# jianwang-mpi/GlobalEgoMocap

Hardware: AMD Instinct MI355X
Metric: optimised windows/sec (10-frame, 15-joint) (higher is better)
Workload: dtype f32

## Files before the change

### globalegomocap_amd/csrc/gem_internal.h

```cpp
#pragma once
#if defined(__HIP_DEVICE_COMPILE__) && !defined(GEM_NO_PACKED_FP32)
#error "compile with: -Xclang -target-feature -Xclang -packed-fp32-ops -DGEM_NO_PACKED_FP32 (__graft_entry__.NO_PACKED_FP32)"
#endif

#include <hip/hip_runtime.h>
#include <stdint.h>
#include <atomic>
#include <set>
#include <string>
#include <vector>

#include "../../include/gem_hip.h"

namespace gem {

constexpr int PAD = 64;
constexpr float LEAKY_SLOPE = 0.01f;
constexpr double BN_EPS = 1e-5;
constexpr int MAX_HIST = 128;
constexpr int MAXJ_ERR = GEM_MAX_JOINTS;
constexpr int N_LOG = 1 << 16;
constexpr int TRACE_ROUNDS = 64;

inline int pad64(int x) { return (x + PAD - 1) / PAD * PAD; }
// ... 88 lines not shown
    int *perm2 = nullptr, *slot_of2 = nullptr;
    int* n_log = nullptr;
    long log_pos = 0;
    int done_phase = 3;
    int dbg_slots = -1, dbg_B = 0, dbg_round = 0;
    long dbg_log0 = 0;
    std::vector<void*> allocs;
};

enum Repack {
    REPACK_NONE = 0,
    REPACK_KERNEL = 1,
    REPACK_FUSED = 2,
    REPACK_ATOMIC = 3
};

struct RoundSet {
    int* n_active = nullptr;
    int* perm = nullptr;
    int* slot_of = nullptr;
    int *next_perm = nullptr, *next_slot_of = nullptr, *next_count = nullptr;
    long log_idx = -1;
    double* trace = nullptr;
};

struct GemmOpts {
    const RoundSet* rs = nullptr;
    const int* row_map = nullptr;
    SlabSrc* defer = nullptr;
    int* repack_log = nullptr;
    GemmOpts() {}
    GemmOpts(std::nullptr_t) {}
    GemmOpts(const RoundSet* rs_, const int* row_map_, SlabSrc* defer_ = nullptr, int* repack_log_ = nullptr)
        : rs(rs_), row_map(row_map_), defer(defer_), repack_log(repack_log_) {}
};

template <typename T>
inline int dev_alloc(std::vector<void*>& owner, T** p, size_t n) {
    void* q = nullptr;
    if (!hip_ok(hipMalloc(&q, (n ? n : 1) * sizeof(T)), "hipMalloc")) return 1;
    owner.push_back(q);
    *p = static_cast<T*>(q);
    return hip_ok(hipMemset(q, 0, (n ? n : 1) * sizeof(T)), "hipMemset") ? 0 : 1;
}
template <typename T>
inline int upload(std::vector<void*>& owner, T** p, const std::vector<T>& v) {
// ... 122 lines not shown
        const DynSplit d = dyn_split(*s.m_dev, 64, s.CT, s.dyn_W, s.n_tiles, s.ldc);
        nslab = d.SK;
        stride = d.slab;
    }
}
bool rows_can_fuse_compaction(const gem_handle* h, const Layer& L, int lda, int ldc, int B, bool slabs);
int launch_splitk_reduce(gem_handle* h, int epi, int nslab, size_t slab, const float* bias, const float* aux, float* C, int M, int N,
                         int ldc, const int* m_dev, hipStream_t s, int dyn_W = 0, int n_tiles = 0);
int launch_gemm_bf16(gem_handle* h, const Layer& L, int epi, int nprod, const float* A, int lda, const float* aux, float* Cout,
                     int ldc, int M, int T, hipStream_t s, const GemmOpts& o);

enum Narrow {
    NARROW_BATCHED = 0,
    NARROW_TAIL_F32 = 1,
    NARROW_TAIL_BF16 = 2
};
struct Route {
    int precision = 0;
    Narrow narrow = NARROW_BATCHED;
    bool front = false;
    int tail_wgs = 0;
    int tail_cap = 0;
    Repack repack = REPACK_KERNEL;
};
enum Call { CALL_DECODE = 0, CALL_EVALUATE = 1, CALL_ROUNDS = 2 };
Route plan_route(const gem_handle* h, int stage, int B, Call call);

struct EnergyArgs;
int evaluate_bf16(gem_handle* h, const Route& rt, int stage, int B, const EnergyArgs& ea, hipStream_t s, bool forward_only, const RoundSet* rs,
                  SlabSrc* grad);
int launch_f32_to_bf16(const float* src, uint16_t* dst, size_t n, hipStream_t s);
int launch_f32_split_bf16(const float* src, uint16_t* hi, uint16_t* lo, size_t n, hipStream_t s);

int launch_pack_pose(const float* src, float* dst, int rows, int C, hipStream_t s);
int launch_unpack_pose(const float* src, float* dst, int rows, int C, hipStream_t s);
int launch_reparam(const float* mulv, const float* eps, float* mu, float* logvar, float* z, float* z2, int B, int D, int Dp,
                   hipStream_t s);
int launch_pad_latent(const float* z, float* zp, int B, int D, int Dp, hipStream_t s);
int launch_unpad_latent(const float* zp, float* z, int B, int D, int Dp, hipStream_t s);

struct EnergyArgs {
    const float* Xp;
    const float* X0;
    const float* heat;
    const int32_t* frame0;
    const float* mean_bone;
// ... 1 lines not shown
    uint16_t* dXp_b;
    double* f;
    double* parts;
    float w3d, ws, wb, wv, wr;
    double dw3d, dws, dwb, dwv, dwr;
    int T, J, H, W, n_poly;
    float poly[GEM_MAX_POLY];
    float cx, cy;
    const int* parents;
    const int* children;
    int* tex_key;
    float* tex_val;
    const int* n_dev;
    const int* perm;
};
int launch_energy(gem_handle* h, const EnergyArgs& a, int B, hipStream_t s);

constexpr int TAIL_MAX_LAYERS = 6;
struct TailLayerDev { const float* w4; const float* bias; int K, N; };
struct TailArgs {
    int n, B, G, forward_only, escr, mask_first;
    int waves, rows;
    int maxnt;
    SlabSrc in_slab;
    const float* in_bias;
    int in_bias_ld;
    long long* dbg_ts;
    TailLayerDev fwd[TAIL_MAX_LAYERS], bwd[TAIL_MAX_LAYERS];
    const float* a_in;
    float* g_out;
    uint16_t* g_out_b;
    float* Xp;
    int off_act[TAIL_MAX_LAYERS + 1], ld_act[TAIL_MAX_LAYERS + 1], off_g[2], ld_g, off_red, off_escr, off_zero, off_pre;
    EnergyArgs e;
};
size_t plan_tail(const std::vector<Layer>& dec, int start, int T, int J, TailArgs* out, bool shared = false);
void fill_tail_args(const gem_handle* h, const StageNet& net, const Route& rt, int B, bool forward_only, const SlabSrc& in_slab,
                    const EnergyArgs& ea, const RoundSet* rs, TailArgs* ta);
size_t plan_tail_for(const gem_handle* h, const std::vector<Layer>& dec, int start, int wgs, TailArgs* out);

constexpr int TB_MAX_LAYERS = 6;
struct TailB16Layer { int K, N; const float* bias; };
struct TailB16Args {
    int n, B, G, nrt, forward_only, mask_first;
    SlabSrc in_slab;
    const float* in_bias;
// ... 46 lines not shown
```

### globalegomocap_amd/csrc/gemm_f32.hip

```cpp
#include <cstdio>
#include <cstdlib>

#include "gem_internal.h"
#include "gemm_glds.h"
#include "gemm_rows.h"

namespace gem {

typedef float f32x16 __attribute__((ext_vector_type(16)));
typedef float f32x4 __attribute__((ext_vector_type(4)));
typedef int i32x8 __attribute__((ext_vector_type(8)));

constexpr int BK_MIN = 32;

#ifdef GEM_TRACE
__device__ long long* g_gemm_trace = nullptr;
#define GEM_TRACE_MARK(slot_)                                                                            \
    if (g_gemm_trace && threadIdx.x == 0)                                                                \
        g_gemm_trace[4 * (blockIdx.x + gridDim.x * (blockIdx.y + gridDim.y * blockIdx.z)) + (slot_)] = wall_clock64();
#else
#define GEM_TRACE_MARK(slot_)
#endif

template <int TAPS, int EPI, int RM, int RN, int TAG, int BK>
// ... 305 lines not shown
    a.n_split = 1; a.tiles_per_split = TAPS * (L.K / 32); a.slab_stride = 0;
    const int grid = ((M + BM - 1) / BM) * (L.N / BN);
    note_kernel(h, reinterpret_cast<const void*>(k));
    hipLaunchKernelGGL(k, dim3(grid), dim3(256), smem, s, a);
    GEM_HIP(hipGetLastError());
    return 0;
}

template <int S, int RT, bool FUSE>
static int launch_rows_as(gem_handle* h, const Layer& L, const float* A, int lda, float* C, int ldc, int M, hipStream_t s,
                          const GemmOpts& o, const rows::Plan& p, bool direct, bool with_bias, bool lrelu) {
    auto k = rows::gemm_rows_kernel<S, RT, FUSE>;
    static PerDeviceOnce once;
    if (once.need(h->cfg.device))
        GEM_HIP(hipFuncSetAttribute(reinterpret_cast<const void*>(k), hipFuncAttributeMaxDynamicSharedMemorySize,
                                    S * rows::Geometry<RT>::STAGE_BYTES));
    Workspace& w = h->ws;
    rows::Args a{};
    a.A = A; a.W = L.w; a.bias = direct && with_bias ? L.bias : nullptr; a.lrelu = lrelu ? 1 : 0; a.C = direct ? C : w.splitk;
    a.m_dev = o.rs ? o.rs->n_active : nullptr;
    a.row_map = o.row_map;
    a.lda = lda; a.ldc = ldc; a.M = M; a.N = L.N; a.K = L.K;
    a.n_rb = p.n_rb; a.n_split = p.n_split; a.tiles_per_split = p.per; a.slab_stride = (size_t)M * ldc;
    if (FUSE) {
        a.phase_arr = w.phase; a.n_windows = M; a.done_phase = w.done_phase; a.T = h->T;
        a.perm_out = o.rs->perm; a.slot_of_out = o.rs->slot_of; a.n_active_out = o.rs->n_active; a.log_slot = o.repack_log;
    }
    const int grid = p.n_rb * (L.N / rows::BN) * p.n_split;
    note_kernel(h, reinterpret_cast<const void*>(k));
    hipLaunchKernelGGL(k, dim3(grid), dim3(256), (size_t)S * rows::Geometry<RT>::STAGE_BYTES, s, a);
    GEM_HIP(hipGetLastError());
    return 0;
}

static bool rows_plan(const gem_handle* h, const Layer& L, int lda, int ldc, int M, bool slabs, rows::Plan* out, bool* use8) {
    if (M < 48 || L.N % rows::BN != 0 || L.K % rows::BK != 0 || (size_t)h->ws.Bmax * lda * 4 >= ((size_t)1 << 32) ||
        (size_t)L.N * L.K * 4 >= ((size_t)1 << 32))
        return false;
    const rows::Plan p5 = rows::plan(M, L.N, L.K, 5, h->n_cu, slabs, h->ws.splitk_elems, ldc);
    const rows::Plan p8 = rows::plan(M, L.N, L.K, 8, h->n_cu, slabs, h->ws.splitk_elems, ldc);
    *use8 = p8.n_rb > 0 && (p5.n_rb == 0 || p8.cost < p5.cost - 1e-9);
    *out = *use8 ? p8 : p5;
    return out->n_rb != 0 && out->fill >= 0.75;
}

bool rows_can_fuse_compaction(const gem_handle* h, const Layer& L, int lda, int ldc, int B, bool slabs) {
// ... 96 lines not shown
```

### globalegomocap_amd/csrc/gemm_rows.h

```cpp
#pragma once
#include <hip/hip_runtime.h>
#include <stdint.h>
#include <type_traits>

namespace gem {
namespace rows {

typedef float f32x4 __attribute__((ext_vector_type(4)));

constexpr int BN = 64;
constexpr int BK = 64;
constexpr int ROW_BYTES = BK * 4;

struct Args {
    const float* A;
    const float* W;
    const float* bias;
    int lrelu;
    float* C;
    const int* m_dev;
    const int* row_map;
    int lda, ldc, M, N, K;
    const int* phase_arr;
    int n_windows, done_phase, T;
    int* perm_out;
    int* slot_of_out;
    int* n_active_out;
    int* log_slot;
    int n_rb;
    int n_split, tiles_per_split;
    size_t slab_stride;
};

template <int RT>
struct Geometry {
    static constexpr int A_BYTES = RT * 16 * ROW_BYTES, B_BYTES = BN * ROW_BYTES, STAGE_BYTES = A_BYTES + B_BYTES;
    static constexpr int A_INSTR = A_BYTES / 1024 / 4, B_INSTR = B_BYTES / 1024 / 4;
    static constexpr int PIECES = A_INSTR + B_INSTR;
    static_assert(A_BYTES % 4096 == 0, "the A tile must split into whole DMA pieces per wave");
};

#ifndef GEM_ROWS_ABLATE
#define GEM_ROWS_ABLATE 0
#endif

#ifdef GEM_ROWS_CLOCK
__device__ long long g_rows_clock[6];
#endif

constexpr int FUSE_MAX_WINDOWS = 512;

template <int S, int RT, bool FUSE = false>
__device__ __forceinline__ void gemm_rows_body(const Args& a) {
    typedef Geometry<RT> G;
// ... 189 lines not shown
            step(f0, f1, std::integral_constant<int, G::A_INSTR>{});
            for (int t = 1; t < nk; t += 2) {
                step(f1, f0, steady);
                if (t + 1 < nk) step(f0, f1, steady);
            }
        } else {
            for (int t = 0; t < nk; t += 2) {
                step(f0, f1, steady);
                if (t + 1 < nk) step(f1, f0, steady);
            }
        }
#ifdef GEM_ROWS_CLOCK
        const long long w1 = wall_clock64();
        if (blockIdx.x == 8 && tid == 0) { g_rows_clock[0] = clock64() - c0; g_rows_clock[1] = w1 - w0; g_rows_clock[2] = w0 - w_begin; }
#endif
        asm volatile("s_waitcnt vmcnt(0)" ::: "memory");
        __syncthreads();
#pragma unroll
        for (int i = 0; i < 4; ++i)
#pragma unroll
            for (int j = 0; j < NRT; ++j)
                *reinterpret_cast<f32x4*>(smem + ((wave * 4 + i) * NRT + j) * 1024 + lane * 16) = acc[i][j];
        __syncthreads();
        f32x4 bv = {0.f, 0.f, 0.f, 0.f};
        if (a.n_split == 1 && a.bias) bv = *reinterpret_cast<const f32x4*>(a.bias + col + 16 * wave);
#pragma unroll
        for (int j = 0; j < NRT; ++j) {
            f32x4 v = *reinterpret_cast<const f32x4*>(smem + ((0 * 4 + wave) * NRT + j) * 1024 + lane * 16);
#pragma unroll
            for (int w = 1; w < 4; ++w) v += *reinterpret_cast<const f32x4*>(smem + ((w * 4 + wave) * NRT + j) * 1024 + lane * 16);
            const int row = m0 + j * 16 + fr;
            if (row < M) {
                v += bv;
                if (a.lrelu && a.n_split == 1) {
#pragma unroll
                    for (int e = 0; e < 4; ++e) v[e] = v[e] > 0.f ? v[e] : v[e] * 0.01f;
                }
                *reinterpret_cast<f32x4*>(Cb + (size_t)row * a.ldc + col + 16 * wave) = v;
            }
        }
#ifdef GEM_ROWS_CLOCK
        if (blockIdx.x == 8 && tid == 0) g_rows_clock[3] = wall_clock64() - w1;
#endif
    };
    switch (nrt) {
        case 1: body(std::integral_constant<int, 1>{}); break;
        case 2: body(std::integral_constant<int, (RT >= 2 ? 2 : RT)>{}); break;
        case 3: body(std::integral_constant<int, (RT >= 3 ? 3 : RT)>{}); break;
        case 4: body(std::integral_constant<int, (RT >= 4 ? 4 : RT)>{}); break;
        case 5: body(std::integral_constant<int, (RT >= 5 ? 5 : RT)>{}); break;
        case 6: body(std::integral_constant<int, (RT >= 6 ? 6 : RT)>{}); break;
        case 7: body(std::integral_constant<int, (RT >= 7 ? 7 : RT)>{}); break;
        default: body(std::integral_constant<int, RT>{}); break;
    }
}

template <int S, int RT, bool FUSE = false>
__global__ __launch_bounds__(256) void gemm_rows_kernel(const Args a) { gemm_rows_body<S, RT, FUSE>(a); }

struct Plan { int n_rb, n_split, per; double fill, cost; };
inline Plan plan(int M, int N, int K, int rt_max, int n_cu, bool allow_split, size_t slab_capacity_elems, int ldc) {
// ... 22 lines not shown
```

### globalegomocap_amd/csrc/lbfgs.hip

```cpp
#include "gem_internal.h"

namespace gem {

typedef float f32x4 __attribute__((ext_vector_type(4)));

enum { PH_INIT = 0, PH_BRACKET = 1, PH_ZOOM = 2, PH_DONE = 3 };
static_assert(PH_DONE == 3, "Workspace::done_phase (gem_internal.h) names this value for the fused compaction of gemm_rows.h");

struct AdvArgs {
    LbfgsState* state;
    const double* f;
    double* trace;
    const float* gnew;
    float *x, *d, *g, *gp, *bg0, *bg1, *trial, *S, *Y;
    uint16_t* trial_b;
    int* phase_arr;
    const int* slot_of;
    int *next_perm, *next_slot_of, *next_count;
    SlabSrc gslab;
    unsigned long long* clk;
    int Dp, hist_cap;
    gem_lbfgs_opts o;
};

__device__ __forceinline__ double cubic_interpolate(double x1, double f1, double g1, double x2, double f2, double g2,
                                                    bool has_bounds, double lo, double hi) {
    if (!has_bounds) {
        lo = x1 <= x2 ? x1 : x2;
        hi = x1 <= x2 ? x2 : x1;
    }
    const double d1 = g1 + g2 - 3.0 * (f1 - f2) / (x1 - x2);
    const double d2s = d1 * d1 - g1 * g2;
    if (d2s >= 0.0) {
        const double d2 = sqrt(d2s);
        double m;
        if (x1 <= x2) m = x2 - (x2 - x1) * ((g2 + d2 - d1) / (g2 - g1 + 2.0 * d2));
        else m = x1 - (x1 - x2) * ((g1 + d2 - d1) / (g1 - g2 + 2.0 * d2));
        double r = (m > lo) ? m : lo;
        if (!(m == m)) r = m;
        double q = (r < hi) ? r : hi;
        if (!(r == r)) q = r;
        return q;
    }
    return (lo + hi) / 2.0;
// ... 84 lines not shown
                const int e = (tid + NT * i) * 4;
                f32x4 w = {0.f, 0.f, 0.f, 0.f};
                if (FULL || e < Dp) w = *reinterpret_cast<const f32x4*>(p + off + e);
                v[4 * i] = w[0]; v[4 * i + 1] = w[1]; v[4 * i + 2] = w[2]; v[4 * i + 3] = w[3];
            }
        } else {
#pragma unroll
            for (int i = 0; i < EPT; ++i) { const int e = tid + NT * i; v[i] = (FULL || e < Dp) ? p[off + e] : 0.f; }
        }
    };
    auto store = [&](float* p, const float (&v)[EPT]) {
        if constexpr (EPT % 4 == 0) {
#pragma unroll
            for (int i = 0; i < EPT / 4; ++i) {
                const int e = (tid + NT * i) * 4;
                const f32x4 w = {v[4 * i], v[4 * i + 1], v[4 * i + 2], v[4 * i + 3]};
                if (FULL || e < Dp) *reinterpret_cast<f32x4*>(p + off + e) = w;
            }
        } else {
#pragma unroll
            for (int i = 0; i < EPT; ++i) { const int e = tid + NT * i; if (FULL || e < Dp) p[off + e] = v[i]; }
        }
    };
    auto hload = [&](const float* base, int slot, float (&v)[EPT]) {
        const size_t eo = ((size_t)b * a.hist_cap + slot) * Dp;
        if constexpr (!HB) { load(base + eo - off, v); }
        else {
            const uint16_t* q = reinterpret_cast<const uint16_t*>(base) + eo;
            if constexpr (EPT % 4 == 0) {
#pragma unroll
                for (int i = 0; i < EPT / 4; ++i) {
                    const int e = (tid + NT * i) * 4;
                    typedef unsigned int u2 __attribute__((ext_vector_type(2)));
                    u2 w = {0u, 0u};
                    if (FULL || e < Dp) w = *reinterpret_cast<const u2*>(q + e);
                    v[4 * i] = __builtin_bit_cast(float, w[0] << 16); v[4 * i + 1] = __builtin_bit_cast(float, w[0] & 0xFFFF0000u);
                    v[4 * i + 2] = __builtin_bit_cast(float, w[1] << 16); v[4 * i + 3] = __builtin_bit_cast(float, w[1] & 0xFFFF0000u);
                }
            } else {
#pragma unroll
                for (int i = 0; i < EPT; ++i) { const int e = tid + NT * i; v[i] = (FULL || e < Dp) ? __builtin_bit_cast(float, (unsigned)q[e] << 16) : 0.f; }
            }
        }
    };
    auto hstore = [&](float* base, int slot, const float (&v)[EPT]) {
        const size_t eo = ((size_t)b * a.hist_cap + slot) * Dp;
        if constexpr (!HB) { store(base + eo - off, v); }
        else {
            uint16_t* q = reinterpret_cast<uint16_t*>(base) + eo;
            if constexpr (EPT % 4 == 0) {
#pragma unroll
                for (int i = 0; i < EPT / 4; ++i) {
                    const int e = (tid + NT * i) * 4;
                    typedef __bf16 bf4 __attribute__((ext_vector_type(4)));
                    const bf4 w = __builtin_convertvector(f32x4{v[4 * i], v[4 * i + 1], v[4 * i + 2], v[4 * i + 3]}, bf4);
                    if (FULL || e < Dp) *reinterpret_cast<bf4*>(q + e) = w;
                }
            } else {
#pragma unroll
                for (int i = 0; i < EPT; ++i) { const int e = tid + NT * i; if (FULL || e < Dp) q[e] = (uint16_t)(__builtin_bit_cast(unsigned int, (float)(__bf16)v[i]) >> 16); }
            }
        }
    };
    auto store_trial = [&](const float (&v)[EPT]) {
        if (!a.trial_b) store(a.trial, v);
        if (a.trial_b) {
            uint16_t* p = a.trial_b + off;
            if constexpr (EPT % 4 == 0) {
#pragma unroll
                for (int i = 0; i < EPT / 4; ++i) {
                    const int e = (tid + NT * i) * 4;
                    typedef __bf16 bf4 __attribute__((ext_vector_type(4)));
                    const bf4 w = __builtin_convertvector(f32x4{v[4 * i], v[4 * i + 1], v[4 * i + 2], v[4 * i + 3]}, bf4);
                    if (FULL || e < Dp) *reinterpret_cast<bf4*>(p + e) = w;
                }
            } else {
#pragma unroll
                for (int i = 0; i < EPT; ++i) {
                    const int e = tid + NT * i;
                    if (FULL || e < Dp) p[e] = (uint16_t)(__builtin_bit_cast(unsigned int, (float)(__bf16)v[i]) >> 16);
                }
            }
        }
    };
    auto copy = [&](float* dst, const float* src) {
        float tmp[EPT];
        load(src, tmp);
        store(dst, tmp);
// ... 32 lines not shown
            for (int k = 0; k < 8; ++k)
                if (z0 + k < nslab) {
#pragma unroll
                    for (int i = 0; i < EPT; ++i) gn[i] += t[k][i];
                }
        }
        if (nslab <= 0) request_rest();
    } else {
        load(gsrc - off, gn);
        request_rest();
    }
    if (tid < a.hist_cap) { ro_s[tid] = ro_v; cadj_s[tid] = cadj_v; }
    __syncthreads();
    float* BG[2] = {a.bg0, a.bg1};

    bool do_zoom_head = false, do_ls_end = false, do_start_iter = false, finished = false, emit = false;
    bool have_ys = false;

    LB_PROBE(2);
    if (phase == PH_INIT) {
        loss = f_new;
        evals = 1;
        n_iter = 0;
        store(a.g, gn);
#pragma unroll
        for (int i = 0; i < EPT; ++i) gcur[i] = gn[i];
        if (maxabs(gn, 1.f) <= o.tol_grad) finished = true;
        else do_start_iter = true;
    } else {
        const double gtd_new = dot(gn, dv);
        if (phase == PH_BRACKET) {
            if (!first_bracket) ls_iter++;
            first_bracket = 0;
            bool enter_zoom = false;
            if (ls_iter < max_ls) {
                const bool c1 = f_new > (loss + o.c1 * t * gtd) || (ls_iter > 1 && f_new >= f_prev);
                const bool c2 = fabs(gtd_new) <= -o.c2 * gtd;
                const bool c3 = gtd_new >= 0.0;
                if (c1 || (!c2 && c3)) {
                    br_t[0] = t_prev; br_t[1] = t;
                    br_f[0] = f_prev; br_f[1] = f_new;
                    br_gtd[0] = gtd_prev; br_gtd[1] = gtd_new;
                    copy(a.bg0, a.gp);
                    store(a.bg1, gn);
                    ls_done = 0;
                    enter_zoom = true;
                } else if (c2) {
                    br_t[0] = br_t[1] = t;
                    br_f[0] = br_f[1] = f_new;
                    br_gtd[0] = br_gtd[1] = gtd_new;
                    store(a.bg0, gn);
                    ls_done = 1;
                    enter_zoom = true;
                } else {
                    const double lo_b = t + 0.01 * (t - t_prev), hi_b = t * 10.0;
                    const double t_next = cubic_interpolate(t_prev, f_prev, gtd_prev, t, f_new, gtd_new, true, lo_b, hi_b);
                    t_prev = t; f_prev = f_new; gtd_prev = gtd_new;
                    store(a.gp, gn);
                    t = t_next;
                    emit = true;
                }
            } else {
                br_t[0] = 0.0; br_t[1] = t;
                br_f[0] = loss; br_f[1] = f_new;
                br_gtd[0] = gtd; br_gtd[1] = gtd_new;
                copy(a.bg0, a.g);
                store(a.bg1, gn);
                ls_done = 0;
                enter_zoom = true;
            }
            if (enter_zoom) {
                insuf = 0;
                if (br_f[0] <= br_f[1]) { low = 0; high = 1; } else { low = 1; high = 0; }
                do_zoom_head = true;
            }
        } else {
            ls_iter++;
            if (f_new > (loss + o.c1 * t * gtd) || f_new >= br_f[low]) {
                br_t[high] = t; br_f[high] = f_new; br_gtd[high] = gtd_new;
                store(BG[high], gn);
                if (br_f[0] <= br_f[1]) { low = 0; high = 1; } else { low = 1; high = 0; }
// ... 35 lines not shown
            }
            t = tn;
            phase = PH_ZOOM;
            emit = true;
        }
    }

    LB_PROBE(4);
    if (do_ls_end) {
        __syncthreads();
        t = br_t[low];
        loss = br_f[low];
        float bl[EPT], gold[EPT];
        load(BG[low], bl);
        load(a.g, gold);
        const float tf = (float)t;
#pragma unroll
        for (int i = 0; i < EPT; ++i) {
            xv[i] = xv[i] + tf * dv[i];
            yv[i] = bl[i] - gold[i];
            sv[i] = dv[i] * tf;
            gcur[i] = bl[i];
        }
        store(a.x, xv);
        store(a.g, bl);
        evals += ls_evals;
        const double gmax = maxabs(bl, 1.f);
        const double dmax = maxabs(sv, 1.f);
        if (n_iter == o.max_iter || evals >= o.max_eval || gmax <= o.tol_grad || dmax <= o.tol_change ||
            fabs(loss - prev_loss) < o.tol_change) {
            finished = true;
        } else {
            do_start_iter = true;
            have_ys = true;
        }
    }

    LB_PROBE(5);
    bool full_path = false;
    if (do_start_iter) {
        n_iter++;
        if (n_iter == 1) {
#pragma unroll
            for (int i = 0; i < EPT; ++i) dv[i] = -gcur[i];
            H_diag = 1.0;
        } else {
            (void)have_ys;
            auto ring_slot = [&](int k) { return (hist_start + k) & hmask; };
// ... 85 lines not shown
                const int kA = hc - 1 - 2 * p2;
                ld2(kA - 2, kA - 3, sZa, yZa, sZb, yZb);
                dstep1(kA, sXa, yXa, sXb, yXb);
                ld2(kA - 4, kA - 5, sXa, yXa, sXb, yXb);
                if (p2 + 1 < np2) dstep1(kA - 2, sZa, yZa, sZb, yZb);
            }
            __syncthreads();
            const float hd = (float)H_diag;
#pragma unroll
            for (int i = 0; i < EPT; ++i) q[i] *= hd;
            if (hc > 0) ld2(0, 1, sXa, yXa, sXb, yXb);
            for (int p2 = 0; p2 < np2; p2 += 2) {
                const int kA = 2 * p2;
                ld2(kA + 2, kA + 3, sZa, yZa, sZb, yZb);
                dstep2(kA, sXa, yXa, sXb, yXb);
                ld2(kA + 4, kA + 5, sXa, yXa, sXb, yXb);
                if (p2 + 1 < np2) dstep2(kA + 2, sZa, yZa, sZb, yZb);
            }
#pragma unroll
            for (int i = 0; i < EPT; ++i) dv[i] = q[i];
        }
        LB_PROBE(7);
        have_d = true;
        store(a.d, dv);
        prev_loss = loss;
        if (n_iter == 1) {
            float p = 0.f;
#pragma unroll
            for (int i = 0; i < EPT; ++i) p += fabsf(gcur[i]);
            const double l1 = R.sum((double)p);
            const double inv = 1.0 / l1;
            t = (inv < 1.0 ? inv : 1.0) * o.lr;
        } else {
            t = o.lr;
        }
        gtd = dot(gcur, dv);
        if (gtd > -o.tol_change) {
            finished = true;
        } else {
            d_norm = maxabs(dv, 1.f);
            max_ls = o.max_eval - evals;
            ls_iter = 0;
            ls_evals = 0;
            t_prev = 0.0; f_prev = loss; gtd_prev = gtd;
            store(a.gp, gcur);
            phase = PH_BRACKET;
            first_bracket = 1;
            emit = true;
        }
    }

    LB_PROBE(8);
    if (finished) {
        phase = PH_DONE;
        if (!have_x) load(a.x, xv);
        store_trial(xv);
    } else if (emit) {
        if (!have_x) load(a.x, xv);
        if (!have_d) load(a.d, dv);
        const float tf = (float)t;
        float tr[EPT];
#pragma unroll
        for (int i = 0; i < EPT; ++i) tr[i] = xv[i] + tf * dv[i];
        store_trial(tr);
        ls_evals++;
    }
    if (tid == 0) {
        if (a.next_count && phase != PH_DONE) {
// ... 89 lines not shown
    }
}

int launch_lbfgs_debug_read(gem_handle* h, int B, gem_lbfgs_debug_state* out, float* x, float* d, float* trial, hipStream_t s) {
    const Workspace& w = h->ws;
    hipLaunchKernelGGL(lbfgs_debug_read_kernel, dim3(B), dim3(256), 0, s, w.state, out, w.x, w.d, w.trial,
                       h->precision == GEM_PRECISION_BF16 ? w.trial_b : nullptr, x, d, trial, h->D, h->Dp);
    GEM_HIP(hipGetLastError());
    return 0;
}

static AdvArgs make_args(gem_handle* h, const gem_lbfgs_opts& o, const RoundSet& rs, const SlabSrc& grad) {
    Workspace& w = h->ws;
    AdvArgs a;
    a.state = w.state; a.f = w.f; a.gnew = w.dz;
    a.trace = rs.trace;
    a.x = w.x; a.d = w.d; a.g = w.g; a.gp = w.gp; a.bg0 = w.bg0; a.bg1 = w.bg1; a.trial = w.trial; a.S = w.S; a.Y = w.Y;
    a.trial_b = h->precision == GEM_PRECISION_BF16 ? w.trial_b : nullptr;
    a.phase_arr = w.phase;
    a.slot_of = rs.slot_of;
    a.next_perm = rs.next_perm; a.next_slot_of = rs.next_slot_of; a.next_count = rs.next_count;
    a.gslab = grad;
    a.clk = w.lbfgs_clk;
    a.Dp = h->Dp; a.hist_cap = w.hist_cap; a.o = o;
    return a;
}

int launch_lbfgs_init(gem_handle* h, int B, hipStream_t s) {
    const size_t n = (size_t)B * h->Dp;
    hipLaunchKernelGGL(lbfgs_init_kernel, dim3((unsigned)((n + 255) / 256)), dim3(256), 0, s, h->ws.state, h->ws.phase, h->ws.trial, h->ws.x,
                       B, h->Dp);
    GEM_HIP(hipGetLastError());
    return 0;
}

int launch_lbfgs_advance(gem_handle* h, int B, const gem_lbfgs_opts& o, const RoundSet& rs, const SlabSrc& grad, hipStream_t s) {
    AdvArgs a = make_args(h, o, rs, grad);
    Profile::Rec rec;
    const bool prof = h->prof.on;
    if (prof) {
        GEM_HIP(hipEventCreate(&rec.a)); GEM_HIP(hipEventCreate(&rec.b));
        rec.family = 2; rec.flops = 0;
        GEM_HIP(hipEventRecord(rec.a, s));
    }
    const int ept = (h->Dp + 255) / 256;
    typedef void (*kern_t)(AdvArgs);
// ... 71 lines not shown
```

### globalegomocap_amd/csrc/stage.hip

```cpp
#include <cstring>

#include "gem_internal.h"

namespace gem {

__global__ void fill_u32_kernel(uint32_t* __restrict__ p, uint32_t v, size_t n) {
    const size_t i = (size_t)blockIdx.x * blockDim.x + threadIdx.x;
    if (i < n) p[i] = v;
}
static int launch_fill_u32(uint32_t* p, uint32_t v, size_t n, hipStream_t s) {
    if (!n) return 0;
    hipLaunchKernelGGL(fill_u32_kernel, dim3((unsigned)((n + 255) / 256)), dim3(256), 0, s, p, v, n);
    GEM_HIP(hipGetLastError());
    return 0;
}


Route plan_route(const gem_handle* h, int stage, int B, Call call) {
    const StageNet& net = h->net[stage];
    Route rt;
    rt.precision = h->precision;
    const bool bf16 = h->precision == GEM_PRECISION_BF16, have_tail = net.tail_start >= 1;
    const int tail_g = h->T <= 16 ? 16 / h->T : 1;
    rt.tail_wgs = (B + tail_g - 1) / tail_g;
    if (call == CALL_DECODE) {
        rt.front = !bf16 && net.front.w;
        return rt;
    }
    if (bf16) {
        const char* t16_env = dev_env("GEM_TAIL16");
        const bool batched_narrow = dev_env("GEM_BATCHED_NARROW") != nullptr;
        rt.front = net.front.wb_hi != nullptr;
        rt.tail_cap = 5 * h->n_cu;
        if (have_tail && !batched_narrow) {
            if (net.tb_stream && !(t16_env && t16_env[0] == '0')) rt.narrow = NARROW_TAIL_BF16;
            else if (rt.tail_wgs <= rt.tail_cap) rt.narrow = NARROW_TAIL_F32;
        }
        if (call == CALL_ROUNDS && rt.narrow == NARROW_TAIL_BF16 && rt.front) rt.repack = REPACK_ATOMIC;
        return rt;
    }
    rt.front = net.front.w != nullptr;
    rt.tail_cap = have_tail ? tail_cap_workgroups(h, net.dec, net.tail_start) : 0;
    if (have_tail && rt.tail_wgs <= rt.tail_cap) rt.narrow = NARROW_TAIL_F32;
    if (call == CALL_ROUNDS && rt.narrow == NARROW_TAIL_F32) {
        const Layer& first = rt.front ? net.front : net.dec_in;
        if (rows_can_fuse_compaction(h, first, h->Dp, first.N, B, rt.front)) rt.repack = REPACK_FUSED;
        else if (h->precision == GEM_PRECISION_F32 && rt.front) rt.repack = REPACK_ATOMIC;
    }
    return rt;
}

static RoundSet round_set(Workspace& w, long log0, int k, Repack mode) {
    RoundSet r;
    const bool odd = mode == REPACK_ATOMIC && (k & 1);
    r.perm = odd ? w.perm2 : w.perm;
    r.slot_of = mode == REPACK_NONE ? nullptr : odd ? w.slot_of2 : w.slot_of;
    r.n_active = w.n_active;
    r.log_idx = log0 + k;
    if (mode == REPACK_ATOMIC) {
        r.n_active = w.n_log + (log0 + k) % N_LOG;
        r.next_count = r.n_active + 1;
        r.next_perm = odd ? w.perm : w.perm2;
        r.next_slot_of = odd ? w.slot_of : w.slot_of2;
    }
    r.trace = k < TRACE_ROUNDS ? w.trace + (size_t)k * w.Bmax : nullptr;
    return r;
}

static int begin_rounds(gem_handle* h, int B, int counters, hipStream_t s, long* log0) {
    Workspace& w = h->ws;
// ... 74 lines not shown

static EnergyArgs energy_args(gem_handle* h, const float* X0, const float* heat, const int32_t* frame0, const float* mean_bone,
                              const gem_energy_weights& wt, bool tex) {
    Workspace& w = h->ws;
    EnergyArgs a;
    a.Xp = w.dec_act.back(); a.X0 = X0; a.heat = heat; a.frame0 = frame0; a.mean_bone = mean_bone;
    a.dXp = w.dXp; a.dXp_b = nullptr; a.f = w.f; a.parts = w.parts;
    a.tex_key = tex ? w.tex_key : nullptr; a.tex_val = tex ? w.tex_val : nullptr;
    a.w3d = (float)wt.w3d; a.ws = (float)wt.smooth; a.wb = (float)wt.bone; a.wv = (float)wt.vae; a.wr = (float)wt.reproj;
    a.dw3d = wt.w3d; a.dws = wt.smooth; a.dwb = wt.bone; a.dwv = wt.vae; a.dwr = wt.reproj;
    a.T = h->T; a.J = h->J; a.H = h->cfg.heat_h; a.W = h->cfg.heat_w; a.n_poly = h->cfg.n_poly;
    for (int i = 0; i < GEM_MAX_POLY; ++i) a.poly[i] = i < h->cfg.n_poly ? (float)h->cfg.poly[i] : 0.f;
    a.cx = (float)h->cfg.cx; a.cy = (float)h->cfg.cy;
    a.parents = h->d_parents; a.children = h->d_children;
    a.n_dev = nullptr; a.perm = nullptr;
    return a;
}

void fill_tail_args(const gem_handle* h, const StageNet& net, const Route& rt, int B, bool forward_only, const SlabSrc& in_slab,
                    const EnergyArgs& ea, const RoundSet* rs, TailArgs* ta) {
    const Workspace& w = h->ws;
    const int st = net.tail_start;
    ta->B = B; ta->forward_only = forward_only ? 1 : 0; ta->dbg_ts = nullptr;
    ta->in_slab = in_slab; ta->in_bias = rt.front ? net.front.bias : net.dec[st - 1].bias;
    ta->in_bias_ld = rt.front ? net.dec[0].N : 0;
    for (int i = 0; i < ta->n; ++i) {
        const Layer& f = net.dec[st + i];
        const Layer& g = net.dec_bwd[st + i];
        ta->fwd[i] = TailLayerDev{f.w4, f.bias, f.K, f.N};
        ta->bwd[i] = TailLayerDev{g.w4, nullptr, g.K, g.N};
    }
    ta->a_in = w.dec_act[st - 1];
    ta->Xp = (rs && !forward_only) ? nullptr : w.dec_act.back();
    ta->e = ea;
}

static int evaluate(gem_handle* h, const Route& rt, int stage, int B, const float* zp, const EnergyArgs& ea, hipStream_t s, bool forward_only,
                    const RoundSet* rs, SlabSrc* grad, int* repack_log = nullptr) {
    StageNet& net = h->net[stage];
    Workspace& w = h->ws;
    *grad = SlabSrc{};
    if (rt.precision == GEM_PRECISION_BF16) return evaluate_bf16(h, rt, stage, B, ea, s, forward_only, rs, grad);
    if (rt.narrow == NARROW_BATCHED) {
        if (decoder_forward(h, rt, stage, B, zp, s, rs, repack_log)) return 1;
        if (forward_only) return 0;
        if (launch_energy(h, ea, B, s)) return 1;
// ... 44 lines not shown
    Workspace& w = h->ws;
    const int B = r.B, stage = r.stage;
    hipStream_t s = r.s;
    if (r.wt.reproj != 0.0 && (!r.heat || !r.frame0)) { set_error("optimize: reproj weight != 0 needs heat-maps and frame indices"); return 1; }
    if (check_lbfgs_opts(w, r.opt, "optimize")) return 1;
    r.rounds = r.opt.max_eval + 1;
    w.dbg_slots = -1;
    if (encoder_forward(h, stage, B, r.pose_in, s)) return 1;
    if (launch_reparam(w.mulv, r.eps, nullptr, nullptr, nullptr, w.trial, B, h->D, h->Dp, s)) return 1;
    if (h->precision == GEM_PRECISION_BF16 && launch_f32_to_bf16(w.trial, w.trial_b, (size_t)B * h->Dp, s)) return 1;
    if (launch_lbfgs_init(h, B, s)) return 1;
    r.route = plan_route(h, stage, B, CALL_ROUNDS);
    if (begin_rounds(h, B, r.route.repack == REPACK_ATOMIC ? r.rounds + 1 : 0, s, &r.log0)) return 1;
    const bool tex = h->tex_cache && w.tex_key && r.wt.reproj != 0.0;
    if (tex && launch_fill_u32(reinterpret_cast<uint32_t*>(w.tex_key), 0xFFFFFFFFu, (size_t)B * h->T * h->J, s)) return 1;
    r.ea = energy_args(h, r.pose_in, r.heat, r.frame0, r.mean_bone, r.wt, tex);
    return launch_fill_u32(reinterpret_cast<uint32_t*>(w.trace), 0xFFFFFFFFu, (size_t)TRACE_ROUNDS * w.Bmax * 2, s);
}

static int stage_round(StageRun& r, int k) {
    gem_handle* h = r.h;
    Workspace& w = h->ws;
    const Repack mode = r.route.repack;
    const RoundSet rs = round_set(w, r.log0, k, mode);
    int* repack_log = nullptr;
    if (k > 0 && mode != REPACK_ATOMIC) {
        if (mode == REPACK_FUSED) repack_log = w.n_log + rs.log_idx % N_LOG;
        else if (launch_compact(h, rs, r.B, 0, r.s)) return 1;
        w.log_pos = rs.log_idx + 1;
    }
    r.ea.n_dev = rs.n_active; r.ea.perm = rs.perm;
    SlabSrc grad;
    if (evaluate(h, r.route, r.stage, r.B, w.trial, r.ea, r.s, false, &rs, &grad, repack_log)) return 1;
    return launch_lbfgs_advance(h, r.B, r.opt, rs, grad, r.s);
}

static int stage_finish(StageRun& r) {
    gem_handle* h = r.h;
    Workspace& w = h->ws;
    SlabSrc none;
    if (evaluate(h, r.route, r.stage, r.B, w.trial, energy_args(h, r.pose_in, r.heat, r.frame0, r.mean_bone, r.wt, false), r.s, true, nullptr, &none))
        return 1;
    if (launch_unpack_pose(w.dec_act.back(), r.pose_out, r.B * h->T, h->C, r.s)) return 1;
    if (r.stats && launch_lbfgs_stats(h, r.B, r.stats, r.s)) return 1;
    return 0;
}

// ... 277 lines not shown
```

### globalegomocap_amd/csrc/tail.hip

```cpp
#include <algorithm>

#include "energy_device.h"

namespace gem {

typedef float f32x16 __attribute__((ext_vector_type(16)));
typedef float f32x4 __attribute__((ext_vector_type(4)));

__device__ __forceinline__ float bf16_round(float x) {
    const __bf16 b = (__bf16)x;
    return (float)b;
}

constexpr int TAIL_WAVES = 8;
constexpr int TAIL_THREADS = TAIL_WAVES * 64;
constexpr int TAIL_WAVES_SHARED = 4;

constexpr int TAIL_ROWS = 16;

#ifndef TAIL_PREFETCH_BLOCKS
#define TAIL_PREFETCH_BLOCKS 1
#endif
#ifndef TAIL_RING_DEPTH
#define TAIL_RING_DEPTH 2
// ... 205 lines not shown
template <int NL, int W>
static __global__ __launch_bounds__(64 * W, W == TAIL_WAVES_SHARED ? 3 : 2) void decoder_tail_kernel(TailArgs a) {
    constexpr int THREADS = 64 * W;
    constexpr bool TIGHT = W == TAIL_WAVES_SHARED;
    constexpr int STAGE_U = 2048 / THREADS;
    constexpr int PRE_E = TAIL_THREADS / THREADS;
    extern __shared__ __attribute__((aligned(16))) float lds[];
    const int tid = threadIdx.x, lane = tid & 63, wave = __builtin_amdgcn_readfirstlane(tid >> 6);
    const int T = a.e.T;
    int probe = 0;
#define TAIL_PROBE()                                                                                   \
    if (a.dbg_ts && blockIdx.x == 0 && tid == 0) {                                                     \
        a.dbg_ts[2 * probe] = clock64();                                                               \
        a.dbg_ts[2 * probe + 1] = wall_clock64();                                                      \
        ++probe;                                                                                       \
    }
    const int w0 = blockIdx.x * a.G;
    const int B = a.e.n_dev ? *a.e.n_dev : a.B;
    if (w0 >= B) return;
    const int nwin = min(a.G, B - w0);
    const int R = nwin * T;
    const size_t row0 = (size_t)w0 * T;

    {
        const int K0 = a.fwd[0].K, q4 = K0 / 4, n4 = (TIGHT ? a.rows : TAIL_ROWS) * q4;
        float* dst = lds + a.off_act[0];
        if (a.in_slab.base) {
            int nslab;
            size_t stride;
            slab_layout(a.in_slab, nslab, stride);
            for (int u = 0; u < STAGE_U; ++u) {
                const int i = tid + u * THREADS, r = i / q4, c = (i - r * q4) * 4;
                if (i >= n4) break;
                f32x4 v = {0.f, 0.f, 0.f, 0.f};
                if (r < R) {
                    const float* p = a.in_slab.base + (row0 + r) * K0 + c;
                    for (int z0 = 0; z0 < nslab; z0 += 8) {
                        f32x4 t[8];
#pragma unroll
                        for (int k = 0; k < 8; ++k) t[k] = *reinterpret_cast<const f32x4*>(p + (size_t)min(z0 + k, nslab - 1) * stride);
#pragma unroll
                        for (int k = 0; k < 8; ++k)
                            if (z0 + k < nslab) v += t[k];
                    }
                    v += *reinterpret_cast<const f32x4*>(a.in_bias + (r % T) * a.in_bias_ld + c);
#pragma unroll
                    for (int q = 0; q < 4; ++q) v[q] = v[q] > 0.f ? v[q] : v[q] * LEAKY_SLOPE;
                }
                *reinterpret_cast<f32x4*>(dst + r * a.ld_act[0] + c) = v;
            }
        } else {
            f32x4 v[STAGE_U];
#pragma unroll
            for (int u = 0; u < STAGE_U; ++u) {
                const int i = tid + u * THREADS, r = i / q4, c = (i - r * q4) * 4;
                v[u] = f32x4{0.f, 0.f, 0.f, 0.f};
                if (i < n4 && r < R) v[u] = *reinterpret_cast<const f32x4*>(a.a_in + (row0 + r) * K0 + c);
            }
#pragma unroll
            for (int u = 0; u < STAGE_U; ++u) {
                const int i = tid + u * THREADS, r = i / q4, c = (i - r * q4) * 4;
                if (i < n4) *reinterpret_cast<f32x4*>(dst + r * a.ld_act[0] + c) = v[u];
            }
        }
        if (tid < 64) lds[a.off_zero + tid] = 0.f;
    }
    float pre_x0[PRE_E], pre_mb = 0.f;
    int pre_par = 0, pre_ch[PRE_E];
#pragma unroll
    for (int k = 0; k < PRE_E; ++k) { pre_x0[k] = 0.f; pre_ch[k] = -1; }
    static_assert(MAXJ * MAXJ <= TAIL_THREADS && MAXJ <= 64, "the children table is parked by PRE_E passes of the workgroup");
    const bool pre_on = a.G == 1 && !a.forward_only && T * a.e.J * 3 <= TAIL_THREADS;
    if (pre_on) {
        const int J = a.e.J, n = T * J * 3, bw = a.e.perm ? a.e.perm[w0] : w0;
#pragma unroll
        for (int k = 0; k < PRE_E; ++k) {
            const int e = tid + k * THREADS;
            if (e < n) pre_x0[k] = a.e.X0[(size_t)bw * n + e];
            if (e < J * MAXJ) pre_ch[k] = a.e.children[e];
        }
        if (tid < J) { pre_mb = a.e.mean_bone[(size_t)bw * J + tid]; pre_par = a.e.parents[tid]; }
    }
    TAIL_PROBE();
    __syncthreads();
    TAIL_PROBE();

    TailPre<W, MAXNT> bpre;
    tail_prefetch<W, MAXNT>(a.fwd[0], bpre);
#pragma unroll
    for (int i = 0; i < NL; ++i) {
        const bool last = (i + 1 == NL);
        float* out = lds + a.off_act[i + 1];
        const int ldo = a.ld_act[i + 1];
        float* Xp = last ? a.Xp : nullptr;
        const TailLayerDev nxt = !last ? a.fwd[i + 1 < NL ? i + 1 : i] : a.bwd[NL - 1];
        tail_gemm<W, MAXNT>(lds + a.off_act[i], a.ld_act[i], lds + a.off_zero, a.fwd[i], nxt, !last || !a.forward_only, T, R, bpre,
                  [&](const f32x4& acc, int r0, int col, float bv) {
#pragma unroll
                      for (int e = 0; e < 4; ++e) {
                          float v = acc[e] + bv;
                          if (!last) v = v > 0.f ? v : v * LEAKY_SLOPE;
                          if (!TIGHT || r0 + e < a.rows) out[(r0 + e) * ldo + col] = v;
                          if (Xp && r0 + e < R) Xp[(row0 + r0 + e) * PAD + col] = v;
                      }
                  });
        if (i == 0 && pre_on) {
            const int J = a.e.J, n = T * J * 3;
            float* pre = lds + a.off_pre;
            int* prei = reinterpret_cast<int*>(pre + n + J);
#pragma unroll
            for (int k = 0; k < PRE_E; ++k) {
                const int e = tid + k * THREADS;
                if (e < n) pre[e] = pre_x0[k];
                if (e < J * MAXJ) prei[J + e] = pre_ch[k];
            }
            if (tid < J) { pre[n + tid] = pre_mb; prei[tid] = pre_par; }
        }
        __syncthreads();
        TAIL_PROBE();
    }
    if (a.forward_only) return;

    float* g_cur = lds + a.off_g[0];
    float* g_nxt = lds + a.off_g[1];
    if (a.G == 1) {
        float* scr = lds + a.off_escr;
        const int J = a.e.J, n = T * J * 3;
        const float* pre = lds + a.off_pre;
        const int* prei = reinterpret_cast<const int*>(pre + n + J);
        if (T == 10 && J == 15)
            energy_window<true, THREADS, 10, 15>(a.e, a.e.perm ? a.e.perm[w0] : w0, tid, lds + a.off_act[NL], a.ld_act[NL], scr,
                                                      scr + a.escr, scr + 2 * a.escr, scr + 3 * a.escr, g_cur, a.ld_g, a.fwd[NL - 1].N,
                                                      nullptr, pre_on ? pre : nullptr, pre_on ? pre + n : nullptr, pre_on ? prei : nullptr,
                                                      pre_on ? prei + J : nullptr);
        else
            energy_window<true, THREADS>(a.e, a.e.perm ? a.e.perm[w0] : w0, tid, lds + a.off_act[NL], a.ld_act[NL], scr,
                                              scr + a.escr, scr + 2 * a.escr, scr + 3 * a.escr, g_cur, a.ld_g, a.fwd[NL - 1].N,
                                              nullptr, pre_on ? pre : nullptr, pre_on ? pre + n : nullptr, pre_on ? prei : nullptr,
                                              pre_on ? prei + J : nullptr);
// ... 162 lines not shown
```

Measured before the change: 32430.

## Use write-through buffer stores for handover data and warm tail weights into cache

```diff
diff --git a/globalegomocap_amd/csrc/gem_internal.h b/globalegomocap_amd/csrc/gem_internal.h
--- a/globalegomocap_amd/csrc/gem_internal.h
+++ b/globalegomocap_amd/csrc/gem_internal.h
@@ -134,6 +134,7 @@
     int *next_perm = nullptr, *next_slot_of = nullptr, *next_count = nullptr;
     long log_idx = -1;
     double* trace = nullptr;
+    bool wt = false;
 };
 
 struct GemmOpts {
@@ -302,6 +303,8 @@
     int tail_wgs = 0;
     int tail_cap = 0;
     Repack repack = REPACK_KERNEL;
+    bool handover_wt = false;
+    bool tail_warm = true;
 };
 enum Call { CALL_DECODE = 0, CALL_EVALUATE = 1, CALL_ROUNDS = 2 };
 Route plan_route(const gem_handle* h, int stage, int B, Call call);
@@ -349,6 +352,7 @@
     int n, B, G, forward_only, escr, mask_first;
     int waves, rows;
     int maxnt;
+    int warm;
     SlabSrc in_slab;
     const float* in_bias;
     int in_bias_ld;
diff --git a/globalegomocap_amd/csrc/gemm_f32.hip b/globalegomocap_amd/csrc/gemm_f32.hip
--- a/globalegomocap_amd/csrc/gemm_f32.hip
+++ b/globalegomocap_amd/csrc/gemm_f32.hip
@@ -351,6 +351,7 @@
     a.row_map = o.row_map;
     a.lda = lda; a.ldc = ldc; a.M = M; a.N = L.N; a.K = L.K;
     a.n_rb = p.n_rb; a.n_split = p.n_split; a.tiles_per_split = p.per; a.slab_stride = (size_t)M * ldc;
+    a.wt = o.rs && o.rs->wt && (size_t)M * ldc * 4 < ((size_t)1 << 32);
     if (FUSE) {
         a.phase_arr = w.phase; a.n_windows = M; a.done_phase = w.done_phase; a.T = h->T;
         a.perm_out = o.rs->perm; a.slot_of_out = o.rs->slot_of; a.n_active_out = o.rs->n_active; a.log_slot = o.repack_log;
diff --git a/globalegomocap_amd/csrc/gemm_rows.h b/globalegomocap_amd/csrc/gemm_rows.h
--- a/globalegomocap_amd/csrc/gemm_rows.h
+++ b/globalegomocap_amd/csrc/gemm_rows.h
@@ -2,6 +2,8 @@
 #include <hip/hip_runtime.h>
 #include <stdint.h>
 #include <type_traits>
+
+#include "handover_store.h"
 
 namespace gem {
 namespace rows {
@@ -30,6 +32,7 @@
     int n_rb;
     int n_split, tiles_per_split;
     size_t slab_stride;
+    int wt;
 };
 
 template <int RT>
@@ -265,6 +268,7 @@
             for (int j = 0; j < NRT; ++j)
                 *reinterpret_cast<f32x4*>(smem + ((wave * 4 + i) * NRT + j) * 1024 + lane * 16) = acc[i][j];
         __syncthreads();
+        const WtRange wr = wt_range(Cb + (size_t)m0 * a.ldc, (unsigned)(min(NRT * 16, M - m0) * a.ldc) * 4u);
         f32x4 bv = {0.f, 0.f, 0.f, 0.f};
         if (a.n_split == 1 && a.bias) bv = *reinterpret_cast<const f32x4*>(a.bias + col + 16 * wave);
 #pragma unroll
@@ -279,7 +283,8 @@
 #pragma unroll
                     for (int e = 0; e < 4; ++e) v[e] = v[e] > 0.f ? v[e] : v[e] * 0.01f;
                 }
-                *reinterpret_cast<f32x4*>(Cb + (size_t)row * a.ldc + col + 16 * wave) = v;
+                if (a.wt) wt_store16(wr, (unsigned)((j * 16 + fr) * a.ldc + col + 16 * wave) * 4u, v);
+                else *reinterpret_cast<f32x4*>(Cb + (size_t)row * a.ldc + col + 16 * wave) = v;
             }
         }
 #ifdef GEM_ROWS_CLOCK
diff --git a/globalegomocap_amd/csrc/handover_store.h b/globalegomocap_amd/csrc/handover_store.h
--- /dev/null
+++ b/globalegomocap_amd/csrc/handover_store.h
@@ -0,0 +1,27 @@
+#pragma once
+#include <hip/hip_runtime.h>
+#include <stdint.h>
+
+namespace gem {
+
+typedef float wt_f32x4 __attribute__((ext_vector_type(4)));
+typedef unsigned int wt_u32x4 __attribute__((ext_vector_type(4)));
+
+constexpr int WT_AUX_SC1 = 16;
+
+struct WtRange {
+    __amdgpu_buffer_rsrc_t rsrc;
+};
+
+__device__ __forceinline__ WtRange wt_range(void* base, unsigned bytes) {
+    const uint64_t p = reinterpret_cast<uint64_t>(base);
+    const unsigned lo = __builtin_amdgcn_readfirstlane((unsigned)p), hi = __builtin_amdgcn_readfirstlane((unsigned)(p >> 32));
+    void* q = reinterpret_cast<void*>(((uint64_t)hi << 32) | lo);
+    return WtRange{__builtin_amdgcn_make_buffer_rsrc(q, 0, (int)__builtin_amdgcn_readfirstlane(bytes), 0x00020000)};
+}
+
+__device__ __forceinline__ void wt_store16(const WtRange& r, unsigned byte_off, const wt_f32x4& v) {
+    __builtin_amdgcn_raw_buffer_store_b128(__builtin_bit_cast(wt_u32x4, v), r.rsrc, (int)byte_off, 0, WT_AUX_SC1);
+}
+
+}
diff --git a/globalegomocap_amd/csrc/lbfgs.hip b/globalegomocap_amd/csrc/lbfgs.hip
--- a/globalegomocap_amd/csrc/lbfgs.hip
+++ b/globalegomocap_amd/csrc/lbfgs.hip
@@ -1,4 +1,5 @@
 #include "gem_internal.h"
+#include "handover_store.h"
 
 namespace gem {
 
@@ -20,6 +21,7 @@
     SlabSrc gslab;
     unsigned long long* clk;
     int Dp, hist_cap;
+    int wt;
     gem_lbfgs_opts o;
 };
 
@@ -150,6 +152,20 @@
             for (int i = 0; i < EPT; ++i) { const int e = tid + NT * i; if (FULL || e < Dp) p[off + e] = v[i]; }
         }
     };
+    auto store_out = [&](float* p, const float (&v)[EPT]) {
+        if constexpr (EPT % 4 == 0 && !HB) {
+            if (a.wt) {
+                const WtRange wr = wt_range(p + off, (unsigned)Dp * 4u);
+#pragma unroll
+                for (int i = 0; i < EPT / 4; ++i) {
+                    const int e = (tid + NT * i) * 4;
+                    wt_store16(wr, (unsigned)e * 4u, f32x4{v[4 * i], v[4 * i + 1], v[4 * i + 2], v[4 * i + 3]});
+                }
+                return;
+            }
+        }
+        store(p, v);
+    };
     auto hload = [&](const float* base, int slot, float (&v)[EPT]) {
         const size_t eo = ((size_t)b * a.hist_cap + slot) * Dp;
         if constexpr (!HB) { load(base + eo - off, v); }
@@ -191,7 +207,7 @@
         }
     };
     auto store_trial = [&](const float (&v)[EPT]) {
-        if (!a.trial_b) store(a.trial, v);
+        if (!a.trial_b) store_out(a.trial, v);
         if (a.trial_b) {
             uint16_t* p = a.trial_b + off;
             if constexpr (EPT % 4 == 0) {
@@ -270,7 +286,7 @@
         loss = f_new;
         evals = 1;
         n_iter = 0;
-        store(a.g, gn);
+        store_out(a.g, gn);
 #pragma unroll
         for (int i = 0; i < EPT; ++i) gcur[i] = gn[i];
         if (maxabs(gn, 1.f) <= o.tol_grad) finished = true;
@@ -304,7 +320,7 @@
                     const double lo_b = t + 0.01 * (t - t_prev), hi_b = t * 10.0;
                     const double t_next = cubic_interpolate(t_prev, f_prev, gtd_prev, t, f_new, gtd_new, true, lo_b, hi_b);
                     t_prev = t; f_prev = f_new; gtd_prev = gtd_new;
-                    store(a.gp, gn);
+                    store_out(a.gp, gn);
                     t = t_next;
                     emit = true;
                 }
@@ -386,8 +402,8 @@
             sv[i] = dv[i] * tf;
             gcur[i] = bl[i];
         }
-        store(a.x, xv);
-        store(a.g, bl);
+        store_out(a.x, xv);
+        store_out(a.g, bl);
         evals += ls_evals;
         const double gmax = maxabs(bl, 1.f);
         const double dmax = maxabs(sv, 1.f);
@@ -519,7 +535,7 @@
         }
         LB_PROBE(7);
         have_d = true;
-        store(a.d, dv);
+        store_out(a.d, dv);
         prev_loss = loss;
         if (n_iter == 1) {
             float p = 0.f;
@@ -540,7 +556,7 @@
             ls_iter = 0;
             ls_evals = 0;
             t_prev = 0.0; f_prev = loss; gtd_prev = gtd;
-            store(a.gp, gcur);
+            store_out(a.gp, gcur);
             phase = PH_BRACKET;
             first_bracket = 1;
             emit = true;
@@ -676,6 +692,7 @@
     a.next_perm = rs.next_perm; a.next_slot_of = rs.next_slot_of; a.next_count = rs.next_count;
     a.gslab = grad;
     a.clk = w.lbfgs_clk;
+    a.wt = rs.wt ? 1 : 0;
     a.Dp = h->Dp; a.hist_cap = w.hist_cap; a.o = o;
     return a;
 }
diff --git a/globalegomocap_amd/csrc/stage.hip b/globalegomocap_amd/csrc/stage.hip
--- a/globalegomocap_amd/csrc/stage.hip
+++ b/globalegomocap_amd/csrc/stage.hip
@@ -20,6 +20,7 @@
     const StageNet& net = h->net[stage];
     Route rt;
     rt.precision = h->precision;
+    rt.tail_warm = dev_env("GEM_NO_TAIL_WARM") == nullptr;
     const bool bf16 = h->precision == GEM_PRECISION_BF16, have_tail = net.tail_start >= 1;
     const int tail_g = h->T <= 16 ? 16 / h->T : 1;
     rt.tail_wgs = (B + tail_g - 1) / tail_g;
@@ -46,6 +47,7 @@
         const Layer& first = rt.front ? net.front : net.dec_in;
         if (rows_can_fuse_compaction(h, first, h->Dp, first.N, B, rt.front)) rt.repack = REPACK_FUSED;
         else if (h->precision == GEM_PRECISION_F32 && rt.front) rt.repack = REPACK_ATOMIC;
+        rt.handover_wt = rt.repack == REPACK_FUSED && rt.front && h->precision == GEM_PRECISION_F32 && !dev_env("GEM_NO_WT_STORES");
     }
     return rt;
 }
@@ -166,6 +168,7 @@
     const Workspace& w = h->ws;
     const int st = net.tail_start;
     ta->B = B; ta->forward_only = forward_only ? 1 : 0; ta->dbg_ts = nullptr;
+    ta->warm = rt.tail_warm ? 1 : 0;
     ta->in_slab = in_slab; ta->in_bias = rt.front ? net.front.bias : net.dec[st - 1].bias;
     ta->in_bias_ld = rt.front ? net.dec[0].N : 0;
     for (int i = 0; i < ta->n; ++i) {
@@ -256,7 +259,8 @@
     gem_handle* h = r.h;
     Workspace& w = h->ws;
     const Repack mode = r.route.repack;
-    const RoundSet rs = round_set(w, r.log0, k, mode);
+    RoundSet rs = round_set(w, r.log0, k, mode);
+    rs.wt = r.route.handover_wt;
     int* repack_log = nullptr;
     if (k > 0 && mode != REPACK_ATOMIC) {
         if (mode == REPACK_FUSED) repack_log = w.n_log + rs.log_idx % N_LOG;
diff --git a/globalegomocap_amd/csrc/tail.hip b/globalegomocap_amd/csrc/tail.hip
--- a/globalegomocap_amd/csrc/tail.hip
+++ b/globalegomocap_amd/csrc/tail.hip
@@ -251,6 +251,12 @@
     const int R = nwin * T;
     const size_t row0 = (size_t)w0 * T;
 
+    TailPre<W, MAXNT> bpre;
+    if constexpr (W == TAIL_WAVES) {
+        tail_prefetch<W, MAXNT>(a.fwd[0], bpre);
+        __builtin_amdgcn_sched_barrier(0);
+    }
+
     {
         const int K0 = a.fwd[0].K, q4 = K0 / 4, n4 = (TIGHT ? a.rows : TAIL_ROWS) * q4;
         float* dst = lds + a.off_act[0];
@@ -294,6 +300,27 @@
         }
         if (tid < 64) lds[a.off_zero + tid] = 0.f;
     }
+    constexpr int WARM_U = 2;
+    float warm_v[WARM_U];
+    if constexpr (W == TAIL_WAVES) {
+        const int nwg = (B + a.G - 1) / a.G;
+        const int nx = (nwg - (int)(blockIdx.x & 7) + 7) >> 3;
+#pragma unroll
+        for (int u = 0; u < WARM_U; ++u) {
+            const int l = (((int)blockIdx.x >> 3) + u * nx) * THREADS + tid;
+            const char* p = reinterpret_cast<const char*>(a.fwd[0].w4);
+            int first = 0;
+#pragma unroll
+            for (int i = 1; i < 2 * NL; ++i) {
+                const bool adj = i >= NL;
+                const TailLayerDev L = adj ? a.bwd[i - NL] : a.fwd[i];
+                const int lines = (adj && a.forward_only) || !a.warm ? 0 : 3 * L.K * L.N / 32;
+                if (l >= first && l < first + lines) p = reinterpret_cast<const char*>(L.w4) + (size_t)(l - first) * 128;
+                first += lines;
+            }
+            warm_v[u] = *reinterpret_cast<const float*>(p);
+        }
+    }
     float pre_x0[PRE_E], pre_mb = 0.f;
     int pre_par = 0, pre_ch[PRE_E];
 #pragma unroll
@@ -314,8 +341,7 @@
     __syncthreads();
     TAIL_PROBE();
 
-    TailPre<W, MAXNT> bpre;
-    tail_prefetch<W, MAXNT>(a.fwd[0], bpre);
+    if constexpr (W != TAIL_WAVES) tail_prefetch<W, MAXNT>(a.fwd[0], bpre);
 #pragma unroll
     for (int i = 0; i < NL; ++i) {
         const bool last = (i + 1 == NL);
@@ -344,6 +370,12 @@
                 if (e < J * MAXJ) prei[J + e] = pre_ch[k];
             }
             if (tid < J) { pre[n + tid] = pre_mb; prei[tid] = pre_par; }
+        }
+        if constexpr (W == TAIL_WAVES) {
+            if (i == 0) {
+#pragma unroll
+                for (int u = 0; u < WARM_U; ++u) asm volatile("" ::"v"(warm_v[u]));
+            }
         }
         __syncthreads();
         TAIL_PROBE();
```

New measurement: 32750 (median of 6 runs). Within noise of the previous version (+1.0%).
